# giuliop/AlgoPlonk

Measured on AMD Instinct MI355X. Metric: proofs/sec, higher is better.
Workload: dtype u32x8 (Montgomery Fr/Fp)

## Files before the change

### algoplonk_amd/csrc/apk_api.cpp

```cpp
#include <stdarg.h>
#include <stdio.h>
#include <stdlib.h>
#include <string.h>
#include <atomic>
#include <mutex>
#include <string>
#include <type_traits>

#include <hip/hip_runtime_api.h>

#include "backend.h"
#include "device_sched.h"
#include "ec.h"
#include "kernels_kzg.h"
#include "kernels_kzg_lagrange.h"
#include "plonk_protocol.h"
#include "proof_codec.h"
#include "runtime_env.h"
#include "selftest_ops.h"

namespace apk {

static thread_local std::string g_err;

// ... 490 lines not shown
    if (curve == APK_BLS12_381) return selftest_status(g1_op_t<FrBLS12381, FpBLS12381>(op, p, q, out), "g1", op);
    set_error("unsupported curve: %d", curve);
    return APK_ERR_ARG;
}

int apk_feu_shape(int curve, int field, int* ul, int* ub, uint32_t* headroom) {
    if (!ul || !ub || !headroom) { set_error("null argument"); return APK_ERR_ARG; }
    if (curve == APK_BN254) { field ? feu_shape_t<FpBN254>(ul, ub, headroom) : feu_shape_t<FrBN254>(ul, ub, headroom); return APK_OK; }
    if (curve == APK_BLS12_381) { field ? feu_shape_t<FpBLS12381>(ul, ub, headroom) : feu_shape_t<FrBLS12381>(ul, ub, headroom); return APK_OK; }
    set_error("unsupported curve: %d", curve);
    return APK_ERR_ARG;
}

int apk_host_feu_op(int curve, int field, int op, uint64_t count, const void* in, void* out) {
    if (count && (!in || !out)) { set_error("null argument"); return APK_ERR_ARG; }
    const uint32_t* i = static_cast<const uint32_t*>(in);
    uint32_t* o = static_cast<uint32_t*>(out);
    if (curve == APK_BN254) return field ? host_feu_batch<FpBN254>(op, count, i, o) : host_feu_batch<FrBN254>(op, count, i, o);
    if (curve == APK_BLS12_381) return field ? host_feu_batch<FpBLS12381>(op, count, i, o) : host_feu_batch<FrBLS12381>(op, count, i, o);
    set_error("unsupported curve: %d", curve);
    return APK_ERR_ARG;
}

int apk_device_fe_op(int curve, int field, int op, int device, uint64_t count, const void* a, const void* b, void* out) {
    if (count && (!a || !b || !out)) { set_error("null argument"); return APK_ERR_ARG; }
    if (!seam_args(curve, count, (op >= 0 && op <= 4) || (op >= 10 && op <= 14), op, "field")) return APK_ERR_ARG;
    if (count == 0) return APK_OK;
    runtime_checkpoint();
    return curve == APK_BN254 ? fe_op_device_bn254(device, field, op, count, a, b, out) : fe_op_device_bls12381(device, field, op, count, a, b, out);
}

int apk_device_feu_op(int curve, int field, int op, int device, uint64_t count, const void* in, void* out) {
    if (count && (!in || !out)) { set_error("null argument"); return APK_ERR_ARG; }
    if (!seam_args(curve, count, op >= 0 && op <= 29, op, "unsaturated")) return APK_ERR_ARG;
    if (count == 0) return APK_OK;
    runtime_checkpoint();
    return curve == APK_BN254 ? feu_op_device_bn254(device, field, op, count, in, out) : feu_op_device_bls12381(device, field, op, count, in, out);
}

int apk_device_g1_op(int curve, int op, int device, uint64_t count, const void* p, const void* q, void* out) {
    const bool unary = op == 2 || op == 21;
    if (count && (!p || !out || (!unary && !q))) { set_error("null argument"); return APK_ERR_ARG; }
    if (!seam_args(curve, count, (op >= 0 && op <= 3) || (op >= 10 && op <= 14) || op == 20 || op == 21, op, "g1")) return APK_ERR_ARG;
    if (count == 0) return APK_OK;
    runtime_checkpoint();
    return curve == APK_BN254 ? g1_op_device_bn254(device, op, count, p, q, out) : g1_op_device_bls12381(device, op, count, p, q, out);
}

int apk_g1_sum(int curve, const void* points, uint64_t count, void* out) {
    if (!out || (count && !points)) { set_error("null argument"); return APK_ERR_ARG; }
    if (curve == APK_BN254) return g1_sum_t<FpBN254>(points, count, out);
    if (curve == APK_BLS12_381) return g1_sum_t<FpBLS12381>(points, count, out);
    set_error("unsupported curve: %d", curve);
    return APK_ERR_ARG;
}

int apk_fe_from_be(int curve, int field, const uint8_t* be, void* out) {
    if (!be || !out) { set_error("null argument"); return APK_ERR_ARG; }
    return host_fe_from_be(curve, field, be, out);
}
int apk_fe_to_be(int curve, int field, const void* in, uint8_t* be) {
    if (!be || !in) { set_error("null argument"); return APK_ERR_ARG; }
    return host_fe_to_be(curve, field, in, be);
}

int apk_marshal_proof(const apk_proof* p, uint8_t* out, size_t cap, size_t* len) {
    if (!p || !out || !len) { set_error("null argument"); return APK_ERR_ARG; }
// ... 30 lines not shown
```

### algoplonk_amd/csrc/backend_impl.h

```cpp
#pragma once
#include <hip/hip_runtime.h>
#include <algorithm>
#include <atomic>
#include <chrono>
#include <condition_variable>
#include <memory>
#include <new>
#include <mutex>
#include <string.h>
#include <time.h>
#include <vector>

#include "backend.h"
#include "dev_buf.h"
#include "slot_pinned.h"
#include "msm_run.h"
#include "kzg_run.h"
#include "kernels_ntt.h"
#include "kernels_poly.h"
#include "gang_kernel.h"
#include "kernels_setup.h"
#include "host_msm.h"
#include "slot_gate.h"
#include "gang.h"
// ... 209 lines not shown
        const int log_n = (which ? (int)log_n_ + 2 : (int)log_n_) - sub_log;
        const Fr* tw = which ? (inverse ? ptr<Fr>(twi_4n_) : ptr<Fr>(tw_4n_)) : (inverse ? ptr<Fr>(twi_n_) : ptr<Fr>(twu_n_));
        if (ntt_twu_) tw = which ? (inverse ? ptr<Fr>(twi_4n_x_) : ptr<Fr>(tw_4n_x_)) : (inverse ? ptr<Fr>(twi_n_x_) : ptr<Fr>(twu_n_x_));
        static const int tile_env = env_int("APK_NTT_TILE_LOG", 0, 0, NTT_TILE_LOG);
        static const int stages_env = env_int("APK_NTT_STAGES", 0, 0, NTT_TILE_LOG);
        int tile_log = log_n <= 19 ? 9 : 10;
        int max_s = log_n <= 19 ? 7 : 9;
        if (tile_env) tile_log = tile_env;
        if (stages_env) max_s = stages_env;
        if (tile_log > log_n) tile_log = log_n;
        if (max_s > tile_log) max_s = tile_log;
        const int passes = (log_n + max_s - 1) / max_s;
        bool busy_now = false, busy_foreign = false;
        if (slots_.size() > 2 && log_n >= 17 && log_n <= 19) busy_now = device_load_over(1, &busy_foreign);
        NttBatch nb{};
        for (int i = 0; i < count; i++) { nb.in[i] = ins[i]; nb.out[i] = outs[i]; nb.in_len[i] = in_lens[i]; }
        hipEvent_t e0 = nullptr, e1 = nullptr;
        Slot* owner = nullptr;
        for (Slot* s : slots_) if (s->own_stream == st || (s->side && s->side == st)) owner = s;
        if (passes > 1) {
            if (!owner || log_n > 29) { set_error("ntt: no workspace for this stream"); return APK_ERR_STATE; }
            for (int i = 0; i < count; i++) nb.wide[i] = ptr<FeU<FRP>>(owner->ntt_wide) + ((size_t)i << log_n);
        }
        Slot* timed = stats_on_ ? owner : nullptr;
        if (timed) { e0 = timed->ev2; e1 = timed->ev3; HIPCHK(hipEventRecord(e0, st)); }
        int t0 = 0;
        for (int p = 0; p < passes; p++) {
            int s = (log_n - t0 + (passes - p) - 1) / (passes - p);
            NttPassArgs a;
            a.log_n = log_n; a.tile_log = tile_log; a.t0 = t0; a.t1 = t0 + s;
            a.first = (p == 0); a.last = (p == passes - 1);
            a.out_len = out_len;
            a.tw_shift = sub_log;
            const dim3 grid(1u << (log_n - tile_log), count);
            const size_t lds = ((size_t)1 << tile_log) * sizeof(FeU<FRP>);
            static const int r4_env = env_int("APK_NTT_RADIX4", -1, -1, 1);
            a.radix4 = r4_env >= 0 ? r4_env : (log_n > 19 || (log_n >= 17 && busy_now) ? 1 : 0);
            if (p == 0) { path(P_NTT_SEQ); if (a.radix4) { path(P_NTT_R4); if (r4_env < 0 && log_n <= 19) { path(P_NTT_R4_LOAD); if (busy_foreign) path(P_DEVICE_LOAD); } } }
            static const int thr_env = env_int("APK_NTT_THREADS", 0, 0, NTT_THREADS) & ~63;
            uint32_t threads = NTT_THREADS;
            if (a.radix4) {
                threads = (1u << tile_log) / 4;
                if (threads < 64) threads = 64;
                if (threads > (uint32_t)NTT_THREADS) threads = NTT_THREADS;
            }
            if (thr_env) threads = (uint32_t)thr_env;
            if (ntt_twu_) ntt_pass_kernel<FRP, true><<<grid, threads, lds, st>>>(nb, tw, pre, post, scale, a);
            else ntt_pass_kernel<FRP, false><<<grid, threads, lds, st>>>(nb, tw, pre, post, scale, a);
            KCHK();
            t0 += s;
        }
        if (timed) {
            HIPCHK(hipEventRecord(e1, st));
            HIPCHK(hipEventSynchronize(e1));
            float ms = 0;
            HIPCHK(hipEventElapsedTime(&ms, e0, e1));
            std::lock_guard<std::mutex> g(stats_mu_);
            stats_.ntt_ms += ms;
            stats_.ntt_elements += ((uint64_t)1 << log_n) * count;
        }
        return APK_OK;
    }
    int run_ntt(hipStream_t st, int which, bool inverse, const Fr* in, Fr* out, uint32_t in_len, uint32_t out_len,
                const Fr* pre, const Fr* post, const Fr* scale, int sub_log = 0) {
        return run_ntt_batch(st, which, inverse, 1, &in, &out, &in_len, out_len, pre, post, scale, sub_log);
    }
    int coset_eval(hipStream_t st, int count, const Fr* const* ins, const uint32_t* lens, Fr* const* outs, int cls = 0) {
        if (!sc_.on()) return run_ntt_batch(st, 1, false, count, ins, outs, lens, n4_, ptr<Fr>(coset_pre_), nullptr, nullptr);
        return run_ntt_batch(st, 1, false, count, ins, outs, lens, n4_ >> sc_.glog, ptr<Fr>(sc_.pre[cls]), nullptr, nullptr, sc_.glog);
    }
    int inv_ntt_n(hipStream_t st, const Fr* in, Fr* out) { return run_ntt(st, 0, true, in, out, n_, n_, nullptr, nullptr, ptr<Fr>(scales_)); }
    int coset_ntt_4n(hipStream_t st, const Fr* in, uint32_t len, Fr* out) {
        return run_ntt(st, 1, false, in, out, len, n4_, ptr<Fr>(coset_pre_), nullptr, nullptr);
    }

    int build_lagrange_table(hipStream_t st, const Aff* d_srs, const void* h_lagrange) {
        DevBuf lag;
        CHK(lag.alloc((size_t)(n_ + 3) * sizeof(Aff)));
        if (h_lagrange) HIPCHK(hipMemcpyAsync(lag.p, h_lagrange, (size_t)n_ * sizeof(Aff), hipMemcpyHostToDevice, st));
        else CHK((g1_to_lagrange_dev<FRP, FPP>(d_srs, n_, ptr<Aff>(lag), st)));
        HIPCHK(hipMemcpyAsync(ptr<Aff>(lag) + n_, lag_dk_, sizeof lag_dk_, hipMemcpyHostToDevice, st));
// ... 475 lines not shown
    }
    void drain(Slot* s) {
        if (s->stream) (void)hipStreamSynchronize(s->stream);
        if (s->side_pending && s->side) { (void)hipStreamSynchronize(s->side); s->side_pending = false; }
        (void)hipGetLastError();
    }
    void release(Slot* s, bool ok) {
        if (!ok) drain(s);
        if (s->side_pending) { s->side_pending = false; if (s->own_stream) (void)hipStreamWaitEvent(s->own_stream, s->ev_side, 0); }
        s->own_stream = s->stream = nullptr;
        gate_.release(s->index);
    }
    struct SlotGuard {
        CurveBackend* b; Slot* s; bool ok = false;
        SlotGuard(CurveBackend* b_) : b(b_), s(b_->acquire()) {}
        ~SlotGuard() { b->release(s, ok); }
    };
    struct MaybeGuard {
        CurveBackend* b; Slot* s; bool owned; bool ok = false;
        static Slot* own(CurveBackend* b) { return std::count(b->slots_.begin(), b->slots_.end(), hook_slot()) ? hook_slot() : nullptr; }
        MaybeGuard(CurveBackend* b_) : b(b_), s(own(b_)), owned(s == nullptr) { if (owned) s = b->acquire(); }
        ~MaybeGuard() { if (owned) b->release(s, ok); }
    };
    static bool is_device_ptr(const void* p) {
        hipPointerAttribute_t at{};
        const bool dev = hipPointerGetAttributes(&at, p) == hipSuccess && at.type == hipMemoryTypeDevice;
        if (!dev) (void)hipGetLastError();
        return dev;
    }

    int powers(hipStream_t st, Fr* out, uint32_t count, const Fr& w, const Fr& scale) {
        PowersBatch<FRP> pb{};
        pb.out[0] = out; pb.w[0] = w; pb.scale[0] = scale;
        return klaunch<PowersK<FRP>, 256>(st, dim3(cdiv(cdiv(count, 8), 256), 1), 256, 0, pb, count);
    }
    int powers_batch(hipStream_t st, int k, Fr* const* outs, const Fr* ws, uint32_t count) {
        PowersBatch<FRP> pb{};
        for (int i = 0; i < k; i++) { pb.out[i] = outs[i]; pb.w[i] = ws[i]; pb.scale[i] = Fr::one(); }
        return klaunch<PowersK<FRP>, 256>(st, dim3(cdiv(cdiv(count, 8), 256), k), 256, 0, pb, count);
    }

    int choose_window(int requested, int log_size, int slots = 1) {
        msm_ctx_ = msm_plan_context(FRP::BITS, FPP::N, msm_bases_, log_size, slots, requested, msm_knobs_from_env());
        if (msm_ctx_.rc != APK_OK) { set_error("%s", msm_ctx_.message); return msm_ctx_.rc; }
        return APK_OK;
    }

    int init_msm_only(int device, const void* bases, uint64_t count, int msm_window) override {
        if (!bases || count == 0 || count >= (1ull << 27)) { set_error("msm context: bad base count"); return APK_ERR_ARG; }
        int ndev = 0;
        hipError_t e = hipGetDeviceCount(&ndev);
        if (e != hipSuccess || ndev == 0) { set_error("no HIP device available (%s); libapk has no CPU fallback", e == hipSuccess ? "0 devices" : hipGetErrorString(e)); return APK_ERR_HIP; }
        if (device < 0 || device >= ndev) { set_error("device %d out of range (%d devices)", device, ndev); return APK_ERR_ARG; }
        device_ = device;
        HIPCHK(hipSetDevice(device_));
        { int cus = 0; if (hipDeviceGetAttribute(&cus, hipDeviceAttributeMultiprocessorCount, device_) == hipSuccess && cus > 0) simds_ = 4u * (uint32_t)cus; }
        msm_only_ = true;
        ws_batch_ = 1;
        msm_bases_ = (uint32_t)count;
        n_ = (uint32_t)count;
        int lg = 0;
        while ((1ull << lg) < count) lg++;
        CHK(choose_window(msm_window, lg));
        CHK(set_sort_lds_limits<FRP>(msm_ctx_));
        DevBuf srs;
        CHK(srs.alloc(count * sizeof(Aff)));
        HIPCHK(hipMemcpy(srs.p, bases, count * sizeof(Aff), hipMemcpyHostToDevice));
        CHK((build_tables<FRP, FPP>(nullptr, msm_ctx_, ptr<Aff>(srs), (uint32_t)count, tab_can_)));
        HIPCHK(hipDeviceSynchronize());
        Slot* s = new Slot();
        s->index = slots_.size();
        slots_.push_back(s);
// ... 39 lines not shown
        n_ = (uint32_t)d->n;
        n4_ = 4 * n_;
        log_n_ = 0;
        while ((1u << log_n_) < n_) log_n_++;
        nb_public_ = d->nb_public;
        nb_commit_ = d->nb_commitments;
        for (uint32_t k = 0; k < nb_commit_; k++) {
            cci_[k] = d->commitment_constraint_index[k];
            if ((uint64_t)nb_public_ + cci_[k] >= n_) { set_error("commitment_constraint_index[%u] = %u: row %llu is outside the domain (n = %u)", k, cci_[k], (unsigned long long)nb_public_ + cci_[k], n_); return APK_ERR_ARG; }
        }
        msm_bases_ = n_ + 3;
        CHK(choose_window(d->msm_window, (int)log_n_, d->slots));
        Fr root = root_of_unity();
        const int adicity = FRP::ADICITY;
        omega4_ = root;
        for (int i = 0; i < adicity - (int)log_n_ - 2; i++) omega4_ = Fr::sqr(omega4_);
        omega_ = Fr::sqr(Fr::sqr(omega4_));
        omega_inv_ = Fr::inv(omega_);
        omega4_inv_ = Fr::inv(omega4_);
        shift_ = fr_u64(FRP::COSET_SHIFT);
        shift_inv_ = Fr::inv(shift_);
        n_inv_ = Fr::inv(fr_u64(n_));
        n4_inv_ = Fr::inv(fr_u64(n4_));
        {
            Fr sn = Fr::pow_u64(shift_, n_);
            Fr i4 = Fr::pow_u64(omega4_, n_);
            Fr cur = sn;
            for (int k = 0; k < 4; k++) { zh_inv_[k] = Fr::inv(cur - Fr::one()); cur = cur * i4; }
        }
        hipStream_t st = nullptr;
        const size_t fn = (size_t)n_ * sizeof(Fr), f4 = (size_t)n4_ * sizeof(Fr);
        CHK(tw_n_.alloc(fn / 2)); CHK(twi_n_.alloc(fn / 2)); CHK(tw_4n_.alloc(f4 / 2)); CHK(twi_4n_.alloc(f4 / 2));
        const Fr ru = fr_u64(32);
        HIPCHK(hipFuncSetAttribute(reinterpret_cast<const void*>(&ntt_pass_kernel<FRP, false>), hipFuncAttributeMaxDynamicSharedMemorySize,
                                   (int)(((size_t)1 << NTT_TILE_LOG) * sizeof(FeU<FRP>))));
        HIPCHK(hipFuncSetAttribute(reinterpret_cast<const void*>(&ntt_pass_kernel<FRP, true>), hipFuncAttributeMaxDynamicSharedMemorySize,
                                   (int)(((size_t)1 << NTT_TILE_LOG) * sizeof(FeU<FRP>))));
        CHK(twu_n_.alloc(fn / 2));
        CHK(powers(st, ptr<Fr>(tw_n_), n_ / 2, omega_, Fr::one()));
        CHK(powers(st, ptr<Fr>(twu_n_), n_ / 2, omega_, ru));
        CHK(powers(st, ptr<Fr>(twi_n_), n_ / 2, omega_inv_, ru));
        CHK(powers(st, ptr<Fr>(tw_4n_), n4_ / 2, omega4_, ru));
        CHK(powers(st, ptr<Fr>(twi_4n_), n4_ / 2, omega4_inv_, ru));
        if (env_int("APK_NTT_TWU", 0, 0, 1)) {
            struct { DevBuf* in; DevBuf* out; uint32_t count; } tabs[4] = {{&twu_n_, &twu_n_x_, n_ / 2}, {&twi_n_, &twi_n_x_, n_ / 2},
                                                                            {&tw_4n_, &tw_4n_x_, n4_ / 2}, {&twi_4n_, &twi_4n_x_, n4_ / 2}};
            for (auto& t : tabs) {
                CHK(t.out->alloc((size_t)t.count * sizeof(FeU<FRP>)));
                unpack_table_kernel<FRP><<<cdiv(t.count, 256), 256, 0, st>>>(ptr<Fr>(*t.in), ptr<FeU<FRP>>(*t.out), t.count);
                KCHK();
            }
            ntt_twu_ = true;
        }
        CHK(coset_pre_.alloc((size_t)(n_ + 4) * sizeof(Fr)));
        CHK(powers(st, ptr<Fr>(coset_pre_), n_ + 4, shift_, ru));
        CHK(coset_post_inv_.alloc(f4));
        CHK(powers(st, ptr<Fr>(coset_post_inv_), n4_, shift_inv_, n4_inv_ * ru));
        CHK(scales_.alloc(2 * sizeof(Fr)));
        {
            Fr sc[2] = {n_inv_ * ru, n4_inv_ * ru};
            HIPCHK(hipMemcpy(scales_.p, sc, sizeof sc, hipMemcpyHostToDevice));
        }
        CHK(x4_.alloc(f4));
        CHK(powers(st, ptr<Fr>(x4_), n4_, omega4_, shift_));
        DevBuf srs;
        CHK(srs.alloc((size_t)(n_ + 3) * sizeof(Aff)));
        HIPCHK(hipMemcpy(srs.p, d->srs_g1, (size_t)(n_ + 3) * sizeof(Aff), hipMemcpyHostToDevice));
        CHK((build_tables<FRP, FPP>(st, msm_ctx_, ptr<Aff>(srs), n_ + 3, tab_can_)));
        wires_lag_mode_ = env_int("APK_WIRES_LAGRANGE", -1, -1, 1);
        {
// ... 801 lines not shown
        for (size_t i = 0; i < lin_terms.size(); i++) {
            if (i == LT_QK || (lin_h_done && i >= LT_H1 && i <= LT_H3) || (host_fixed && (i <= LT_QO || i == LT_S3))) continue;
            lp[cnt] = lin_terms[i].com; lk[cnt] = lin_terms[i].coef; cnt++;
        }
        const auto t_lc = std::chrono::steady_clock::now();
        XYZZ<FPP, Fe64<FPP>> sum = host_lincomb_sum<FRP, FPP>(lp, lk, cnt, pool, host_glv);
        if (host_fixed) {
            const Fr fk[5] = {lin_terms[LT_QL].coef, lin_terms[LT_QR].coef, lin_terms[LT_QM].coef, lin_terms[LT_QO].coef, lin_terms[LT_S3].coef};
            vk_fixed_.template accumulate<FRP>(sum, fk);
        }
        if (lin_h_done) sum.add(lin_h);
        {
            using F64 = Fe64<FPP>;
            sum.madd(Affine<FPP, F64>{F64::from(key.qk.x), F64::from(key.qk.y)});
        }
        lin_com = host_xyzz_to_affine<FPP>(sum);
        if (stats_on_) lincomb_ms += std::chrono::duration<double, std::milli>(std::chrono::steady_clock::now() - t_lc).count();
    }
    memcpy(out->zshift_value, &e.zw, sizeof(Fr));
    Fr claimed[6 + APK_MAX_COMMITMENTS] = {lin_sc.lin_z, e.l, e.r, e.o, e.s1, e.s2};
    for (uint32_t k = 0; k < nb_commit_; k++) claimed[6 + k] = e.qcp[k];
    for (uint32_t i = 0; i < 6 + nb_commit_; i++) memcpy(out->claimed_values[i], &claimed[i], sizeof(Fr));
    const Fr gk = Proto::gamma_kzg(zeta, lin_com, lro[0], lro[1], lro[2], key, lin_sc.lin_z, e, gk_raw);
    {
        LinCombArgs<FRP> lc{};
        int c = 0;
        for (const LinTerm& t : lin_terms) { lc.f[c] = t.poly; lc.len[c] = t.len; lc.coef[c] = t.coef; c++; }
        Fr acc = gk;
        auto push = [&](const Fr* f, uint32_t len) { lc.f[c] = f; lc.len[c] = len; lc.coef[c] = acc; c++; acc = acc * gk; };
        push(ptr<Fr>(s.cl), n + 2); push(ptr<Fr>(s.cr), n + 2); push(ptr<Fr>(s.co), n + 2);
        push(ptr<Fr>(s_c_[0]), n); push(ptr<Fr>(s_c_[1]), n);
        for (uint32_t k = 0; k < nb_commit_; k++) push(ptr<Fr>(qcp_c_[k]), n);
        lc.count = c; lc.out_len = n + 3;
        {
            const Fr c32 = fr_u64(32);
            for (int k = 0; k < c; k++) lc.coef[k] = lc.coef[k] * c32;
        }
        CHK((klaunch<LincombK<FRP>, POLY_THREADS>(st, cdiv(n + 3, POLY_THREADS), POLY_THREADS, 0, lc, ptr<Fr>(s.folded))));
        CHK(kzg_quotient(s, ptr<Fr>(s.folded), n + 3, ptr<Fr>(s.pw_z), ptr<Fr>(s.pw_zi), z0, ptr<Fr>(s.q1)));
        MsmBatchArgs a{};
        a.batch = 2;
        a.scalars[0] = s.q1.p; a.len[0] = n + 2; a.offset[0] = 0;
        a.scalars[1] = s.q2.p; a.len[1] = n + 2; a.offset[1] = 0;
        CHK(commit(s, tab_can_, 0, a));
    }
    CHK(sync_results(s));
    store_pt(out->zshift_h, hp[1]);
    store_pt(out->batched_h, hp[0]);
    memcpy(out->gamma, &gamma, sizeof(Fr)); memcpy(out->beta, &beta, sizeof(Fr)); memcpy(out->alpha, &alpha, sizeof(Fr));
    memcpy(out->zeta, &zeta, sizeof(Fr)); memcpy(out->gamma_kzg, &gk, sizeof(Fr));
    mark(3);
    in.ok = true;
    guard.ok = true;
    path(P_PROOFS);
    if (stats_on_) {
        double ms = std::chrono::duration<double, std::milli>(std::chrono::steady_clock::now() - t_start).count();
        std::lock_guard<std::mutex> g(stats_mu_);
        stats_.prove_ms += ms;
        stats_.proofs += 1;
        for (int r = 0; r < 4; r++) stats_.round_ms[r] += phase_ms[r];
        stats_.host_lincomb_ms += lincomb_ms;
    }
    return APK_OK;
}

template <class FRP, class FPP>
// ... 37 lines not shown
    CHK(derr.alloc(4));
    HIPCHK(hipMemcpy(din.p, in, count * nb, hipMemcpyHostToDevice));
    HIPCHK(hipMemset(derr.p, 0, 4));
    g1_decompress_kernel<FRP, FPP, CURVE_ID><<<cdiv(count, 256), 256>>>(ptr<uint8_t>(din), (uint32_t)count, ptr<Aff>(dout), ptr<uint32_t>(derr));
    KCHK();
    uint32_t bad = 0;
    HIPCHK(hipMemcpy(&bad, derr.p, 4, hipMemcpyDeviceToHost));
    if (bad) { set_error("%u compressed point(s) are not valid G1 encodings", bad); return APK_ERR_ARG; }
    HIPCHK(hipMemcpy(out, dout.p, count * sizeof(Aff), hipMemcpyDeviceToHost));
    return APK_OK;
}

template <class FRP, class FPP>
int g1_to_lagrange_dev(const Affine<FPP>* d_in, uint64_t n, Affine<FPP>* d_out, hipStream_t st) {
    using Fr = Fe<FRP>;
    using Aff = Affine<FPP>;
    using Pt = XYZZ<FPP>;
    if (n < 2 || (n & (n - 1)) || n > (1ull << 24)) { set_error("ToLagrangeG1: size must be a power of two in [2, 2^24]"); return APK_ERR_ARG; }
    int log_n = 0;
    while ((1ull << log_n) < n) log_n++;
    Fr root;
    for (int i = 0; i < Fr::N; i++) root.l[i] = FRP::root(i);
    Fr w = Fr::to_mont(root);
    for (int i = 0; i < FRP::ADICITY - log_n; i++) w = Fr::sqr(w);
    Fr winv = Fr::inv(w);
    Fr nn = Fr::zero();
    nn.l[0] = (uint32_t)n;
    Fr ninv = Fr::inv(Fr::to_mont(nn));
    DevBuf work, twi;
    CHK(work.alloc(n * sizeof(Pt)));
    CHK(twi.alloc((n / 2 + 1) * sizeof(Fr)));
    PowersBatch<FRP> pb{};
    pb.out[0] = ptr<Fr>(twi); pb.w[0] = winv; pb.scale[0] = Fr::one();
    powers_kernel<FRP><<<dim3(cdiv(cdiv(n / 2, 8), 256), 1), 256, 0, st>>>(pb, (uint32_t)(n / 2));
    KCHK();
    lagrange_load_kernel<FPP><<<cdiv(n, 256), 256, 0, st>>>(d_in, (uint32_t)n, log_n, ptr<Pt>(work));
    KCHK();
    for (int t = 0; t < log_n; t++) {
        lagrange_stage_kernel<FRP, FPP><<<cdiv(n / 2, 128), 128, 0, st>>>(ptr<Pt>(work), ptr<Fr>(twi), (uint32_t)n, log_n, t);
        KCHK();
    }
    lagrange_finish_kernel<FRP, FPP><<<cdiv(n, 128), 128, 0, st>>>(ptr<Pt>(work), (uint32_t)n, ninv, d_out);
    KCHK();
    HIPCHK(hipStreamSynchronize(st));
    return APK_OK;
}

template <class FRP, class FPP>
int g1_to_lagrange_impl(int device, const void* points, uint64_t n, void* out) {
    using Aff = Affine<FPP>;
    if (n < 2 || (n & (n - 1)) || n > (1ull << 24)) { set_error("ToLagrangeG1: size must be a power of two in [2, 2^24]"); return APK_ERR_ARG; }
    CHK(pick_device(device));
    DevBuf din, dout;
    CHK(din.alloc(n * sizeof(Aff)));
    CHK(dout.alloc(n * sizeof(Aff)));
    HIPCHK(hipMemcpy(din.p, points, n * sizeof(Aff), hipMemcpyHostToDevice));
    CHK((g1_to_lagrange_dev<FRP, FPP>(ptr<Aff>(din), n, ptr<Aff>(dout))));
    HIPCHK(hipMemcpy(out, dout.p, n * sizeof(Aff), hipMemcpyDeviceToHost));
    return APK_OK;
}

template <class P>
__global__ void __launch_bounds__(256) fe_op_kernel(int op, uint32_t count, const Fe<P>* __restrict__ a, const Fe<P>* __restrict__ b,
                                                    Fe<P>* __restrict__ out) {
    const uint32_t i = blockIdx.x * blockDim.x + threadIdx.x;
    if (i < count) (void)fe_op_t<P>(op, a + i, b + i, out + i);
}
// ... 77 lines not shown
```

### algoplonk_amd/csrc/ffu.h

```cpp
#pragma once
#include "ff.h"
#include "ffu_asm.h"

template <class P>
struct FeU {
    static constexpr int L = P::UL;
    static constexpr int B = P::UB;
    static constexpr uint32_t MASK = (1u << B) - 1u;
    static constexpr int N = P::N;
    uint32_t l[L];

    APK_HD static FeU zero() {
        FeU r;
#pragma unroll
        for (int i = 0; i < L; i++) r.l[i] = 0;
        return r;
    }
    APK_HD static FeU one() {
        FeU r;
#pragma unroll
        for (int i = 0; i < L; i++) r.l[i] = P::uone(i);
        return r;
    }
    APK_HD bool is_zero() const {
// ... 231 lines not shown
        }
#pragma unroll
        for (int k = L; k < 2 * L - 1; k++) {
#pragma unroll
            for (int i = k - L + 1; i < L; i++) {
                acc += (uint64_t)a.l[i] * b.l[k - i];
                acc += (uint64_t)c.l[i] * d.l[k - i];
            }
#pragma unroll
            for (int i = k - L + 1; i < L; i++) acc += (uint64_t)m[i] * P::umod(k - i);
            r.l[k - L] = (uint32_t)acc & MASK;
            acc >>= B;
        }
        r.l[L - 1] = (uint32_t)acc;
        return r;
    }

    template <uint32_t K>
    APK_HD static FeU canon(const FeU& a) {
        FeU d;
        uint32_t borrow = 0;
#pragma unroll
        for (int i = 0; i < L; i++) {
            uint32_t t = a.l[i] - kp<K>(i) - borrow;
            borrow = t >> 31;
            d.l[i] = i == L - 1 ? t : (t & MASK);
        }
        FeU r;
#pragma unroll
        for (int i = 0; i < L; i++) r.l[i] = borrow ? a.l[i] : d.l[i];
        if constexpr (K > 1) return canon<K / 2>(r);
        else return r;
    }
    APK_HD bool is_zero_mod_p() const {
        uint32_t z = 0, e = 0;
#pragma unroll
        for (int i = 0; i < L; i++) { z |= l[i]; e |= l[i] ^ P::umod(i); }
        return z == 0 || e == 0;
    }

    APK_HD static FeU unpack(const uint32_t* w) {
        FeU r;
#pragma unroll
        for (int i = 0; i < L; i++) {
            const int bit = i * B, j = bit >> 5, s = bit & 31;
            uint32_t v = j < N ? (w[j] >> s) : 0u;
            if (s + B > 32 && j + 1 < N) v |= w[j + 1] << (32 - s);
            r.l[i] = v & MASK;
        }
        return r;
    }
    APK_HD void pack(uint32_t* w) const {
#pragma unroll
        for (int j = 0; j < N; j++) {
            uint32_t v = 0;
#pragma unroll
            for (int i = 0; i < L; i++) {
                const int lo = i * B - j * 32;
                if (lo > -B && lo < 32) v |= lo >= 0 ? (l[i] << lo) : (l[i] >> (-lo));
            }
            w[j] = v;
        }
    }

    APK_HD static FeU from_fe(const Fe<P>& x) {
        FeU c;
// ... 19 lines not shown
```

### algoplonk_amd/csrc/kernels_ntt.h

```cpp
#pragma once
#include "ff.h"
#include "ffu.h"

namespace apk {

constexpr int NTT_TILE_LOG = 11;
constexpr int NTT_PASS_BITS = 10;
constexpr int NTT_THREADS = 256;

__device__ __forceinline__ uint32_t bitrev32(uint32_t x, int bits) { return __brev(x) >> (32 - bits); }

constexpr int NTT_MAX_BATCH = 4;
constexpr int NTT_ARGS_MAX = 16;
struct NttBatch {
    const void* in[NTT_ARGS_MAX];
    void* out[NTT_ARGS_MAX];
    uint32_t in_len[NTT_ARGS_MAX];
    void* wide[NTT_ARGS_MAX];
};

struct NttPassArgs {
    int log_n;
    int tile_log;
    int t0, t1;
    int first, last;
    uint32_t out_len;
    int radix4;
    int tw_shift;
};

template <class FR, bool TWU = false>
__global__ void __launch_bounds__(NTT_THREADS) ntt_pass_kernel(NttBatch nb, const Fe<FR>* __restrict__ tw,
                                                               const Fe<FR>* __restrict__ pre,
                                                               const Fe<FR>* __restrict__ post,
                                                               const Fe<FR>* __restrict__ scale,
                                                               NttPassArgs a) {
    wave_priority<APK_PRIO_FR>();
    using Fr = Fe<FR>;
    using Fu = FeU<FR>;
    static_assert(Fu::HEADROOM >= 64, "values reach (4 + 2 log2 N) p < 64 p over the stages of a transform (N <= 2^29)");
    extern __shared__ __attribute__((aligned(16))) unsigned char smem_raw[];
    Fu* sm = reinterpret_cast<Fu*>(smem_raw);
    const Fu* __restrict__ twu = reinterpret_cast<const Fu*>(tw);
    auto twiddle = [&](uint32_t idx) -> Fu {
        if constexpr (TWU) return twu[idx];
        else { Fr w = tw[idx]; return Fu::unpack(w.l); }
    };
    Fr* __restrict__ out = reinterpret_cast<Fr*>(nb.out[blockIdx.y]);
    const Fr* __restrict__ in = reinterpret_cast<const Fr*>(nb.in[blockIdx.y]);
    Fu* __restrict__ wide = reinterpret_cast<Fu*>(nb.wide[blockIdx.y]);
    const uint32_t in_len = nb.in_len[blockIdx.y];
    const int s = a.t1 - a.t0;
    const int tile_log = a.tile_log;
    const int clog = tile_log - s;
    const uint32_t C = 1u << clog;
    const uint32_t tile_elems = 1u << tile_log;
    const uint32_t g0 = blockIdx.x << clog;
    const uint32_t lomask = (1u << a.t0) - 1u;

    const uint32_t NT = blockDim.x;
    for (uint32_t e = threadIdx.x; e < tile_elems; e += NT) {
        uint32_t c = e & (C - 1), mid = e >> clog;
        uint32_t g = g0 + c;
        uint32_t idx = ((g >> a.t0) << a.t1) | (mid << a.t0) | (g & lomask);
        Fu v;
        if (a.first) {
            uint32_t src = bitrev32(idx, a.log_n);
            if (src < in_len) {
                Fr raw = in[src];
                v = Fu::unpack(raw.l);
                if (pre) { Fr pw = pre[src]; v = Fu::mul_nr(Fu::unpack(pw.l), v); }
                if (in_len > (1u << a.log_n)) {
                    for (uint32_t s2 = src + (1u << a.log_n); s2 < in_len; s2 += 1u << a.log_n) {
                        Fr raw2 = in[s2];
                        Fu v2 = Fu::unpack(raw2.l);
                        if (pre) { Fr pw = pre[s2]; v2 = Fu::mul_nr(Fu::unpack(pw.l), v2); }
                        v = Fu::add_n(v, v2);
                    }
                    v = Fu::template canon<4>(v);
                }
            } else {
                v = Fu::zero();
            }
        } else {
            v = wide[idx];
        }
        sm[e] = v;
    }
    __syncthreads();
    int q = 0;
    const bool padded = a.first && in_len < (1u << a.log_n);
    const uint32_t nq = tile_elems >> 2;
    for (; a.radix4 && q + 2 <= s; q += 2) {
        const int t = a.t0 + q;
        for (uint32_t u4 = threadIdx.x; u4 < nq; u4 += NT) {
            const uint32_t c = u4 & (C - 1), pr = u4 >> clog;
            const uint32_t low = pr & ((1u << q) - 1u);
            const uint32_t m00 = ((pr >> q) << (q + 2)) | low;
            const uint32_t g = g0 + c;
            const uint32_t imod = (low << a.t0) | (g & lomask);
            const uint32_t e00 = (m00 << clog) | c, st1 = 1u << (q + clog);
            const uint32_t e01 = e00 + st1, e10 = e00 + 2 * st1, e11 = e01 + 2 * st1;
            Fu x0 = sm[e00], x1 = sm[e01], x2 = sm[e10], x3 = sm[e11];
            if (padded && q == 0 && x1.is_zero() && x2.is_zero() && x3.is_zero()) {
                sm[e01] = x0; sm[e10] = x0; sm[e11] = x0;
                continue;
            }
            if (t != 0) {
                const Fu w1 = twiddle((imod << (a.log_n - 1 - t)) << a.tw_shift);
                x1 = Fu::mul_nr(w1, x1);
                x3 = Fu::mul_nr(w1, x3);
            }
            const Fu y0 = Fu::add_n(x0, x1);
            const Fu y1 = Fu::template sub_k<2>(x0, x1);
            Fu y2 = Fu::add_n(x2, x3);
            Fu y3 = Fu::template sub_k<2>(x2, x3);
            const uint32_t k2 = imod << (a.log_n - 2 - t);
            {
                y3 = Fu::mul_nr(twiddle((k2 + (1u << (a.log_n - 2))) << a.tw_shift), y3);
            }
            if (t != 0) {
                y2 = Fu::mul_nr(twiddle(k2 << a.tw_shift), y2);
                sm[e00] = Fu::add_n(y0, y2);
                sm[e10] = Fu::template sub_k<2>(y0, y2);
            } else {
                sm[e00] = Fu::add_n(y0, y2);
                sm[e10] = Fu::template sub_k<4>(y0, y2);
            }
            sm[e01] = Fu::add_n(y1, y3);
            sm[e11] = Fu::template sub_k<2>(y1, y3);
        }
        __syncthreads();
    }
    const uint32_t nbf = tile_elems >> 1;
    for (; q < s; q++) {
        const int t = a.t0 + q;
        for (uint32_t bf = threadIdx.x; bf < nbf; bf += NT) {
            uint32_t c = bf & (C - 1), pr = bf >> clog;
            uint32_t low = pr & ((1u << q) - 1u);
            uint32_t mid0 = ((pr >> q) << (q + 1)) | low;
            uint32_t mid1 = mid0 | (1u << q);
            uint32_t g = g0 + c;
            uint32_t imod = (low << a.t0) | (g & lomask);
            uint32_t tidx = (imod << (a.log_n - 1 - t)) << a.tw_shift;
            uint32_t e0 = (mid0 << clog) | c, e1 = (mid1 << clog) | c;
            Fu u = sm[e0];
            Fu v = sm[e1];
            if (t != 0 && !(padded && v.is_zero())) v = Fu::mul_nr(twiddle(tidx), v);
            sm[e0] = Fu::add_n(u, v);
            sm[e1] = Fu::template sub_k<2>(u, v);
        }
        __syncthreads();
    }
    for (uint32_t e = threadIdx.x; e < tile_elems; e += NT) {
        uint32_t c = e & (C - 1), mid = e >> clog;
        uint32_t g = g0 + c;
        uint32_t idx = ((g >> a.t0) << a.t1) | (mid << a.t0) | (g & lomask);
        Fu v = sm[e];
        if (!a.last) { wide[idx] = v; continue; }
        if (idx >= a.out_len) continue;
        if (post) { Fr pw = post[idx]; v = Fu::mul_nr(Fu::unpack(pw.l), v); }
        if (scale) { Fr sc = scale[0]; v = Fu::mul_nr(Fu::unpack(sc.l), v); }
        v = (post || scale) ? Fu::template canon<1>(v) : Fu::template canon<32>(v);
        Fr o;
        v.pack(o.l);
        out[idx] = o;
    }
}

template <class FR>
__global__ void __launch_bounds__(256) unpack_table_kernel(const Fe<FR>* __restrict__ in, FeU<FR>* __restrict__ out, uint32_t count) {
    const uint32_t i = blockIdx.x * blockDim.x + threadIdx.x;
    if (i >= count) return;
    Fe<FR> v = in[i];
    out[i] = FeU<FR>::unpack(v.l);
}

constexpr int POWERS_MAX_BATCH = 4;
template <class FR>
struct PowersBatch {
    Fe<FR>* out[POWERS_MAX_BATCH];
    Fe<FR> w[POWERS_MAX_BATCH];
    Fe<FR> scale[POWERS_MAX_BATCH];
};
template <class FR>
struct PowersK {
    static __device__ __forceinline__ void run(PowersBatch<FR> pb, uint32_t count) {
        using Fr = Fe<FR>;
        using U = FeU<FR>;
        constexpr uint32_t PER = 8;
        Fr* __restrict__ out = pb.out[blockIdx.y];
        uint32_t t = blockIdx.x * blockDim.x + threadIdx.x;
        uint32_t start = t * PER;
        if (start >= count) return;
        const U wu = U::from_fe(pb.w[blockIdx.y]);
        U r = U::one();
        bool started = false;
        for (int b = 31; b >= 0; b--) {
            if (started) r = U::sqr(r);
            if ((start >> b) & 1u) { r = started ? U::mul(r, wu) : wu; started = true; }
        }
        Fr first = r.to_fe();
        U cur = U::mul(U::unpack(first.l), U::from_fe(pb.scale[blockIdx.y]));
        for (uint32_t k = 0; k < PER && start + k < count; k++) {
            Fr o;
            cur.pack(o.l);
            out[start + k] = o;
            cur = U::mul(wu, cur);
        }
    }
};
template <class FR>
__global__ void __launch_bounds__(256) powers_kernel(PowersBatch<FR> pb, uint32_t count) { PowersK<FR>::run(pb, count); }

}
```

### algoplonk_amd/csrc/kernels_poly.h

```cpp
#pragma once
#include "ff.h"
#include "ffu.h"

namespace apk {

constexpr int POLY_THREADS = 256;
constexpr int SCAN_PER_THREAD = 8;
constexpr int SCAN_BLOCK = POLY_THREADS * SCAN_PER_THREAD;

template <class FR>
struct Fr4 { Fe<FR> v[4]; };

template <class FR>
__global__ void fill_zero_kernel(Fe<FR>* p, uint32_t count) {
    uint32_t i = blockIdx.x * blockDim.x + threadIdx.x;
    if (i < count) p[i] = Fe<FR>::zero();
}

template <class FR>
struct BlindK {
    static __device__ __forceinline__ void run(Fe<FR>* p, uint32_t n, Fr4<FR> b, int d) {
        int i = threadIdx.x;
        if (i < d) {
            p[i] = p[i] - b.v[i];
// ... 403 lines not shown
template <class FR>
struct DerivePowers { const Fe<FR>* in[2]; Fe<FR>* out[2]; int inverse[2]; };
template <class FR>
struct DerivePowersK {
    static __device__ __forceinline__ void run(DerivePowers<FR> a, const Fe<FR>* __restrict__ twu, uint32_t n, uint32_t count) {
        wave_priority<APK_PRIO_FR>();
        using Fr = Fe<FR>;
        using U = FeU<FR>;
        const uint32_t i = blockIdx.x * blockDim.x + threadIdx.x;
        if (i >= count) return;
        const int p = blockIdx.y;
        uint32_t e = i & (n - 1u);
        if (a.inverse[p]) e = (n - e) & (n - 1u);
        const bool neg = e >= n / 2;
        Fr w = twu[e & (n / 2 - 1u)], v = a.in[p][i];
        U r = U::template canon<1>(U::mul_nr(U::unpack(w.l), U::unpack(v.l)));
        Fr o;
        r.pack(o.l);
        if (neg) o = Fr::neg(o);
        a.out[p][i] = o;
    }
};
template <class FR>
__global__ void __launch_bounds__(POLY_THREADS) derive_powers_kernel(DerivePowers<FR> a, const Fe<FR>* __restrict__ twu, uint32_t n, uint32_t count) { DerivePowersK<FR>::run(a, twu, n, count); }

constexpr int LC_MAX = 20;
template <class FR>
struct LinCombArgs {
    const Fe<FR>* f[LC_MAX];
    uint32_t len[LC_MAX];
    Fe<FR> coef[LC_MAX];
    int count;
    uint32_t out_len;
};

template <class FR>
struct LincombK {
    static __device__ __forceinline__ void run(LinCombArgs<FR> a, Fe<FR>* __restrict__ out) {
        wave_priority<APK_PRIO_FR>();
        using Fr = Fe<FR>;
        using U = FeU<FR>;
        static_assert(U::HEADROOM >= 64 && LC_MAX * 2 <= 64, "the sum of LC_MAX products below 2 r each must stay below 64 r");
        uint32_t i = blockIdx.x * blockDim.x + threadIdx.x;
        if (i >= a.out_len) return;
        U acc = U::zero();
        for (int k = 0; k < a.count; k++)
            if (i < a.len[k]) { Fr v = a.f[k][i]; acc = U::add_n(acc, U::mul_nr(U::unpack(a.coef[k].l), U::unpack(v.l))); }
        const U res = U::template canon<32>(acc);
        Fr w;
        res.pack(w.l);
        out[i] = w;
    }
};
template <class FR>
__global__ void __launch_bounds__(POLY_THREADS) lincomb_kernel(LinCombArgs<FR> a, Fe<FR>* __restrict__ out) { LincombK<FR>::run(a, out); }

template <class FR>
struct DivFinishK {
    static __device__ __forceinline__ void run(const Fe<FR>* __restrict__ suffix,
                                                                  const Fe<FR>* __restrict__ zinv_pw, uint32_t len,
                                                                  Fe<FR>* __restrict__ q) {
        wave_priority<APK_PRIO_FR>();
        uint32_t j = blockIdx.x * blockDim.x + threadIdx.x;
        if (j + 1 >= len) return;
        q[j] = suffix[j + 1] * zinv_pw[j + 1];
    }
};
template <class FR>
__global__ void __launch_bounds__(POLY_THREADS) div_finish_kernel(const Fe<FR>* __restrict__ suffix,
                                                                  const Fe<FR>* __restrict__ zinv_pw, uint32_t len,
                                                                  Fe<FR>* __restrict__ q) { DivFinishK<FR>::run(suffix, zinv_pw, len, q); }

template <int DUMMY>
struct TailNonzeroK {
    static __device__ __forceinline__ void run(const uint4* __restrict__ words, uint32_t count4, uint32_t epoch, uint32_t* __restrict__ flag) {
        uint32_t acc = 0;
        for (uint32_t i = blockIdx.x * blockDim.x + threadIdx.x; i < count4; i += gridDim.x * blockDim.x) {
            const uint4 v = words[i];
            acc |= v.x | v.y | v.z | v.w;
        }
        if (__ballot(acc != 0) != 0 && (threadIdx.x & 63) == 0) *reinterpret_cast<volatile uint32_t*>(flag) = epoch;
// ... 17 lines not shown
```

### algoplonk_amd/csrc/selftest_ops.h

```cpp
#pragma once
#include <string.h>
#include <type_traits>

#include "ec.h"

namespace apk {

enum { SELFTEST_OK = 0, SELFTEST_UNKNOWN_OP = 1, SELFTEST_NO_UNSAT = 2 };

template <class P, class = void> struct HasUnsat : std::false_type {};
template <class P> struct HasUnsat<P, std::void_t<decltype(P::UL)>> : std::true_type {};

template <class P>
APK_HD int fe_op_t(int op, const void* a, const void* b, void* out) {
    using F = Fe<P>;
    F x, y, r;
    memcpy(&x, a, sizeof x);
    if (b) memcpy(&y, b, sizeof y); else y = F::zero();
    switch (op) {
        case 0: r = F::add(x, y); break;
        case 1: r = F::sub(x, y); break;
        case 2: r = F::mul(x, y); break;
        case 3: r = F::inv(x); break;
        case 4: r = F::neg(x); break;
// ... 38 lines not shown
        U a, b, c, d, r = U::zero();
        for (int i = 0; i < L; i++) { a.l[i] = in[i]; b.l[i] = in[L + i]; c.l[i] = in[2 * L + i]; d.l[i] = in[3 * L + i]; }
        switch (op) {
            case 0: r = U::reduce_once(a); break;
            case 1: r = U::add(a, b); break;
            case 2: r = U::sub(a, b); break;
            case 3: r = U::neg(a); break;
            case 4: r = U::mul_nr(a, b); break;
            case 5: r = U::mul(a, b); break;
            case 6: r = U::sqr_nr(a); break;
            case 7: r = U::sqr(a); break;
            case 8: r = U::mul2_nr(a, b, c, d); break;
            case 9: r = U::add_n(a, b); break;
            case 10: r = U::triple_n(a); break;
            case 11: r = U::template sub2_k<4>(a, b, c); break;
            case 12: r = U::template sub_k<1>(a, b); break;
            case 13: r = U::template sub_k<2>(a, b); break;
            case 14: r = U::template sub_k<4>(a, b); break;
            case 15: r = U::template sub_k<6>(a, b); break;
            case 16: r = U::template neg_k<1>(a); break;
            case 17: r = U::template neg_k<2>(a); break;
            case 18: r = U::template neg_k<4>(a); break;
            case 19: r = U::template canon<1>(a); break;
            case 20: r = U::template canon<2>(a); break;
            case 21: r = U::template canon<4>(a); break;
            case 22: r = U::template canon<8>(a); break;
            case 23: r = U::template canon<16>(a); break;
            case 24: r = U::template canon<32>(a); break;
            case 25: r.l[0] = a.is_zero_mod_p() ? 1u : 0u; break;
            case 26: r = U::unpack(in); break;
            case 27: a.pack(r.l); break;
            case 28: { Fe<P> x; memcpy(&x, in, sizeof x); r = U::from_fe(x); break; }
            case 29: { const Fe<P> x = a.to_fe(); memcpy(r.l, &x, sizeof x); break; }
            default: return SELFTEST_UNKNOWN_OP;
        }
        for (int i = 0; i < L; i++) out[i] = r.l[i];
        return SELFTEST_OK;
    } else {
        return SELFTEST_NO_UNSAT;
    }
}

template <class FRP, class FPP>
APK_HD int g1_op_t(int op, const void* p, const void* q, void* out) {
    using A = Affine<FPP>;
    using X = XYZZ<FPP>;
    A a, b, r;
    memcpy(&a, p, sizeof a);
    switch (op) {
        case 0: {
            memcpy(&b, q, sizeof b);
            X acc = X::from_affine(a);
            acc.madd(b);
            r = acc.to_affine();
            break;
        }
        case 1: {
            memcpy(&b, q, sizeof b);
            X acc = X::dbl_affine(a);
            acc.madd(a, true);
            X other = X::dbl_affine(b);
            other.madd(b, true);
            acc.add(other);
            r = acc.to_affine();
            break;
        }
// ... 110 lines not shown
```

Measured before the change: 544.6.

## Add quotient-estimate canonicalization, padded-NTT template split, and adaptive powers walk

```diff
diff --git a/algoplonk_amd/csrc/apk_api.cpp b/algoplonk_amd/csrc/apk_api.cpp
--- a/algoplonk_amd/csrc/apk_api.cpp
+++ b/algoplonk_amd/csrc/apk_api.cpp
@@ -546,7 +546,7 @@
 
 int apk_device_feu_op(int curve, int field, int op, int device, uint64_t count, const void* in, void* out) {
     if (count && (!in || !out)) { set_error("null argument"); return APK_ERR_ARG; }
-    if (!seam_args(curve, count, op >= 0 && op <= 29, op, "unsaturated")) return APK_ERR_ARG;
+    if (!seam_args(curve, count, (op >= 0 && op <= 29) || op == 31, op, "unsaturated")) return APK_ERR_ARG;
     if (count == 0) return APK_OK;
     runtime_checkpoint();
     return curve == APK_BN254 ? feu_op_device_bn254(device, field, op, count, in, out) : feu_op_device_bls12381(device, field, op, count, in, out);
diff --git a/algoplonk_amd/csrc/backend_impl.h b/algoplonk_amd/csrc/backend_impl.h
--- a/algoplonk_amd/csrc/backend_impl.h
+++ b/algoplonk_amd/csrc/backend_impl.h
@@ -265,6 +265,8 @@
             a.first = (p == 0); a.last = (p == passes - 1);
             a.out_len = out_len;
             a.tw_shift = sub_log;
+            static const int est_env = env_int("APK_NTT_CANON_EST", 1, 0, 1);
+            a.canon_est = est_env;
             const dim3 grid(1u << (log_n - tile_log), count);
             const size_t lds = ((size_t)1 << tile_log) * sizeof(FeU<FRP>);
             static const int r4_env = env_int("APK_NTT_RADIX4", -1, -1, 1);
@@ -278,8 +280,16 @@
                 if (threads > (uint32_t)NTT_THREADS) threads = NTT_THREADS;
             }
             if (thr_env) threads = (uint32_t)thr_env;
-            if (ntt_twu_) ntt_pass_kernel<FRP, true><<<grid, threads, lds, st>>>(nb, tw, pre, post, scale, a);
-            else ntt_pass_kernel<FRP, false><<<grid, threads, lds, st>>>(nb, tw, pre, post, scale, a);
+            static const int hoist_env = env_int("APK_NTT_PADDED_HOIST", 1, 0, 1);
+            bool padded = !hoist_env;
+            if (p == 0) for (int i = 0; i < count; i++) if (in_lens[i] < (1u << log_n)) padded = true;
+            if (ntt_twu_) {
+                if (padded) ntt_pass_kernel<FRP, true, true><<<grid, threads, lds, st>>>(nb, tw, pre, post, scale, a);
+                else ntt_pass_kernel<FRP, true, false><<<grid, threads, lds, st>>>(nb, tw, pre, post, scale, a);
+            } else {
+                if (padded) ntt_pass_kernel<FRP, false, true><<<grid, threads, lds, st>>>(nb, tw, pre, post, scale, a);
+                else ntt_pass_kernel<FRP, false, false><<<grid, threads, lds, st>>>(nb, tw, pre, post, scale, a);
+            }
             KCHK();
             t0 += s;
         }
@@ -821,12 +831,16 @@
     int powers(hipStream_t st, Fr* out, uint32_t count, const Fr& w, const Fr& scale) {
         PowersBatch<FRP> pb{};
         pb.out[0] = out; pb.w[0] = w; pb.scale[0] = scale;
-        return klaunch<PowersK<FRP>, 256>(st, dim3(cdiv(cdiv(count, 8), 256), 1), 256, 0, pb, count);
+        return klaunch<PowersK<FRP>, 256>(st, dim3(cdiv(cdiv(count, POWERS_WALK), 256), 1), 256, 0, pb, count, POWERS_WALK);
     }
     int powers_batch(hipStream_t st, int k, Fr* const* outs, const Fr* ws, uint32_t count) {
         PowersBatch<FRP> pb{};
         for (int i = 0; i < k; i++) { pb.out[i] = outs[i]; pb.w[i] = ws[i]; pb.scale[i] = Fr::one(); }
-        return klaunch<PowersK<FRP>, 256>(st, dim3(cdiv(cdiv(count, 8), 256), k), 256, 0, pb, count);
+        static const int walk_env = env_int("APK_POWERS_WALK", -1, -1, (int)POWERS_WALK_MAX);
+        uint32_t per = POWERS_WALK;
+        if (walk_env > 0) per = (uint32_t)walk_env;
+        else if (walk_env < 0 && slots_.size() > 2 && device_load_over(1)) per = POWERS_WALK_LOADED;
+        return klaunch<PowersK<FRP>, 256>(st, dim3(cdiv(cdiv(count, per), 256), k), 256, 0, pb, count, per);
     }
 
     int choose_window(int requested, int log_size, int slots = 1) {
@@ -932,10 +946,9 @@
         const size_t fn = (size_t)n_ * sizeof(Fr), f4 = (size_t)n4_ * sizeof(Fr);
         CHK(tw_n_.alloc(fn / 2)); CHK(twi_n_.alloc(fn / 2)); CHK(tw_4n_.alloc(f4 / 2)); CHK(twi_4n_.alloc(f4 / 2));
         const Fr ru = fr_u64(32);
-        HIPCHK(hipFuncSetAttribute(reinterpret_cast<const void*>(&ntt_pass_kernel<FRP, false>), hipFuncAttributeMaxDynamicSharedMemorySize,
-                                   (int)(((size_t)1 << NTT_TILE_LOG) * sizeof(FeU<FRP>))));
-        HIPCHK(hipFuncSetAttribute(reinterpret_cast<const void*>(&ntt_pass_kernel<FRP, true>), hipFuncAttributeMaxDynamicSharedMemorySize,
-                                   (int)(((size_t)1 << NTT_TILE_LOG) * sizeof(FeU<FRP>))));
+        for (const void* fn_ntt : {reinterpret_cast<const void*>(&ntt_pass_kernel<FRP, false, true>), reinterpret_cast<const void*>(&ntt_pass_kernel<FRP, false, false>),
+                                   reinterpret_cast<const void*>(&ntt_pass_kernel<FRP, true, true>), reinterpret_cast<const void*>(&ntt_pass_kernel<FRP, true, false>)})
+            HIPCHK(hipFuncSetAttribute(fn_ntt, hipFuncAttributeMaxDynamicSharedMemorySize, (int)(((size_t)1 << NTT_TILE_LOG) * sizeof(FeU<FRP>))));
         CHK(twu_n_.alloc(fn / 2));
         CHK(powers(st, ptr<Fr>(tw_n_), n_ / 2, omega_, Fr::one()));
         CHK(powers(st, ptr<Fr>(twu_n_), n_ / 2, omega_, ru));
@@ -1803,6 +1816,8 @@
         push(ptr<Fr>(s_c_[0]), n); push(ptr<Fr>(s_c_[1]), n);
         for (uint32_t k = 0; k < nb_commit_; k++) push(ptr<Fr>(qcp_c_[k]), n);
         lc.count = c; lc.out_len = n + 3;
+        static const int lc_est = env_int("APK_LINCOMB_CANON_EST", 1, 0, 1);
+        lc.canon_est = lc_est;
         {
             const Fr c32 = fr_u64(32);
             for (int k = 0; k < c; k++) lc.coef[k] = lc.coef[k] * c32;
@@ -1906,7 +1921,7 @@
     CHK(twi.alloc((n / 2 + 1) * sizeof(Fr)));
     PowersBatch<FRP> pb{};
     pb.out[0] = ptr<Fr>(twi); pb.w[0] = winv; pb.scale[0] = Fr::one();
-    powers_kernel<FRP><<<dim3(cdiv(cdiv(n / 2, 8), 256), 1), 256, 0, st>>>(pb, (uint32_t)(n / 2));
+    powers_kernel<FRP><<<dim3(cdiv(cdiv(n / 2, POWERS_WALK), 256), 1), 256, 0, st>>>(pb, (uint32_t)(n / 2), POWERS_WALK);
     KCHK();
     lagrange_load_kernel<FPP><<<cdiv(n, 256), 256, 0, st>>>(d_in, (uint32_t)n, log_n, ptr<Pt>(work));
     KCHK();
diff --git a/algoplonk_amd/csrc/ffu.h b/algoplonk_amd/csrc/ffu.h
--- a/algoplonk_amd/csrc/ffu.h
+++ b/algoplonk_amd/csrc/ffu.h
@@ -287,6 +287,39 @@
         if constexpr (K > 1) return canon<K / 2>(r);
         else return r;
     }
+    template <uint32_t K2>
+    struct KpTable {
+        uint32_t l[K2][L];
+        constexpr KpTable() : l{} {
+            for (uint32_t j = 0; j < K2; j++) {
+                uint64_t carry = 0;
+                for (int i = 0; i < L; i++) {
+                    const uint64_t t = (uint64_t)j * P::umod(i) + carry;
+                    l[j][i] = i == L - 1 ? (uint32_t)t : (uint32_t)(t & MASK);
+                    carry = t >> B;
+                }
+            }
+        }
+    };
+    template <uint32_t K>
+    APK_HD static FeU canon_est(const FeU& a) {
+        constexpr uint32_t D = P::umod(L - 1) + 1;
+        constexpr uint32_t M = (uint32_t)((1ull << 32) / D);
+        static_assert((uint64_t)2 * K * D <= (1ull << 30), "canon_est: the top limb of a value below 2K*p must stay below 2^30");
+        static_assert((uint64_t)4 * (2 * K + 1) <= D - 1, "canon_est: the estimate must be at most one short");
+        static constexpr KpTable<2 * K> T{};
+        uint32_t q = (uint32_t)(((uint64_t)a.l[L - 1] * M) >> 32);
+        q = q < 2 * K - 1 ? q : 2 * K - 1;
+        FeU d;
+        int32_t carry = 0;
+#pragma unroll
+        for (int i = 0; i < L; i++) {
+            int32_t t = (int32_t)(a.l[i] - T.l[q][i]) + carry;
+            carry = t >> B;
+            d.l[i] = i == L - 1 ? (uint32_t)t : ((uint32_t)t & MASK);
+        }
+        return reduce_once(d);
+    }
     APK_HD bool is_zero_mod_p() const {
         uint32_t z = 0, e = 0;
 #pragma unroll
diff --git a/algoplonk_amd/csrc/kernels_ntt.h b/algoplonk_amd/csrc/kernels_ntt.h
--- a/algoplonk_amd/csrc/kernels_ntt.h
+++ b/algoplonk_amd/csrc/kernels_ntt.h
@@ -27,9 +27,10 @@
     uint32_t out_len;
     int radix4;
     int tw_shift;
-};
-
-template <class FR, bool TWU = false>
+    int canon_est;
+};
+
+template <class FR, bool TWU = false, bool PADDED = true>
 __global__ void __launch_bounds__(NTT_THREADS) ntt_pass_kernel(NttBatch nb, const Fe<FR>* __restrict__ tw,
                                                                const Fe<FR>* __restrict__ pre,
                                                                const Fe<FR>* __restrict__ post,
@@ -89,13 +90,15 @@
     }
     __syncthreads();
     int q = 0;
-    const bool padded = a.first && in_len < (1u << a.log_n);
+    const bool padded = PADDED && a.first && in_len < (1u << a.log_n);
     const uint32_t nq = tile_elems >> 2;
     for (; a.radix4 && q + 2 <= s; q += 2) {
         const int t = a.t0 + q;
+        const int sh1 = a.log_n - 1 - t + a.tw_shift, sh2 = sh1 - 1;
+        const uint32_t quarter = (1u << (a.log_n - 2)) << a.tw_shift, qmask = (1u << q) - 1u;
         for (uint32_t u4 = threadIdx.x; u4 < nq; u4 += NT) {
             const uint32_t c = u4 & (C - 1), pr = u4 >> clog;
-            const uint32_t low = pr & ((1u << q) - 1u);
+            const uint32_t low = pr & qmask;
             const uint32_t m00 = ((pr >> q) << (q + 2)) | low;
             const uint32_t g = g0 + c;
             const uint32_t imod = (low << a.t0) | (g & lomask);
@@ -107,7 +110,7 @@
                 continue;
             }
             if (t != 0) {
-                const Fu w1 = twiddle((imod << (a.log_n - 1 - t)) << a.tw_shift);
+                const Fu w1 = twiddle(imod << sh1);
                 x1 = Fu::mul_nr(w1, x1);
                 x3 = Fu::mul_nr(w1, x3);
             }
@@ -115,12 +118,12 @@
             const Fu y1 = Fu::template sub_k<2>(x0, x1);
             Fu y2 = Fu::add_n(x2, x3);
             Fu y3 = Fu::template sub_k<2>(x2, x3);
-            const uint32_t k2 = imod << (a.log_n - 2 - t);
+            const uint32_t k2 = imod << sh2;
             {
-                y3 = Fu::mul_nr(twiddle((k2 + (1u << (a.log_n - 2))) << a.tw_shift), y3);
+                y3 = Fu::mul_nr(twiddle(k2 + quarter), y3);
             }
             if (t != 0) {
-                y2 = Fu::mul_nr(twiddle(k2 << a.tw_shift), y2);
+                y2 = Fu::mul_nr(twiddle(k2), y2);
                 sm[e00] = Fu::add_n(y0, y2);
                 sm[e10] = Fu::template sub_k<2>(y0, y2);
             } else {
@@ -135,14 +138,16 @@
     const uint32_t nbf = tile_elems >> 1;
     for (; q < s; q++) {
         const int t = a.t0 + q;
+        const int sh = a.log_n - 1 - t + a.tw_shift;
+        const uint32_t qmask = (1u << q) - 1u;
         for (uint32_t bf = threadIdx.x; bf < nbf; bf += NT) {
             uint32_t c = bf & (C - 1), pr = bf >> clog;
-            uint32_t low = pr & ((1u << q) - 1u);
+            uint32_t low = pr & qmask;
             uint32_t mid0 = ((pr >> q) << (q + 1)) | low;
             uint32_t mid1 = mid0 | (1u << q);
             uint32_t g = g0 + c;
             uint32_t imod = (low << a.t0) | (g & lomask);
-            uint32_t tidx = (imod << (a.log_n - 1 - t)) << a.tw_shift;
+            uint32_t tidx = imod << sh;
             uint32_t e0 = (mid0 << clog) | c, e1 = (mid1 << clog) | c;
             Fu u = sm[e0];
             Fu v = sm[e1];
@@ -161,7 +166,7 @@
         if (idx >= a.out_len) continue;
         if (post) { Fr pw = post[idx]; v = Fu::mul_nr(Fu::unpack(pw.l), v); }
         if (scale) { Fr sc = scale[0]; v = Fu::mul_nr(Fu::unpack(sc.l), v); }
-        v = (post || scale) ? Fu::template canon<1>(v) : Fu::template canon<32>(v);
+        v = (post || scale) ? Fu::template canon<1>(v) : a.canon_est ? Fu::template canon_est<32>(v) : Fu::template canon<32>(v);
         Fr o;
         v.pack(o.l);
         out[idx] = o;
@@ -177,6 +182,7 @@
 }
 
 constexpr int POWERS_MAX_BATCH = 4;
+constexpr uint32_t POWERS_WALK = 8, POWERS_WALK_LOADED = 64, POWERS_WALK_MAX = 1024;
 template <class FR>
 struct PowersBatch {
     Fe<FR>* out[POWERS_MAX_BATCH];
@@ -185,14 +191,13 @@
 };
 template <class FR>
 struct PowersK {
-    static __device__ __forceinline__ void run(PowersBatch<FR> pb, uint32_t count) {
+    static __device__ __forceinline__ void run(PowersBatch<FR> pb, uint32_t count, uint32_t per) {
         using Fr = Fe<FR>;
         using U = FeU<FR>;
-        constexpr uint32_t PER = 8;
         Fr* __restrict__ out = pb.out[blockIdx.y];
         uint32_t t = blockIdx.x * blockDim.x + threadIdx.x;
-        uint32_t start = t * PER;
-        if (start >= count) return;
+        if (t >= (count + per - 1) / per) return;
+        uint32_t start = t * per;
         const U wu = U::from_fe(pb.w[blockIdx.y]);
         U r = U::one();
         bool started = false;
@@ -202,7 +207,7 @@
         }
         Fr first = r.to_fe();
         U cur = U::mul(U::unpack(first.l), U::from_fe(pb.scale[blockIdx.y]));
-        for (uint32_t k = 0; k < PER && start + k < count; k++) {
+        for (uint32_t k = 0; k < per && start + k < count; k++) {
             Fr o;
             cur.pack(o.l);
             out[start + k] = o;
@@ -211,6 +216,6 @@
     }
 };
 template <class FR>
-__global__ void __launch_bounds__(256) powers_kernel(PowersBatch<FR> pb, uint32_t count) { PowersK<FR>::run(pb, count); }
+__global__ void __launch_bounds__(256) powers_kernel(PowersBatch<FR> pb, uint32_t count, uint32_t per) { PowersK<FR>::run(pb, count, per); }
 
 }
diff --git a/algoplonk_amd/csrc/kernels_poly.h b/algoplonk_amd/csrc/kernels_poly.h
--- a/algoplonk_amd/csrc/kernels_poly.h
+++ b/algoplonk_amd/csrc/kernels_poly.h
@@ -459,6 +459,7 @@
     Fe<FR> coef[LC_MAX];
     int count;
     uint32_t out_len;
+    int canon_est;
 };
 
 template <class FR>
@@ -473,7 +474,7 @@
         U acc = U::zero();
         for (int k = 0; k < a.count; k++)
             if (i < a.len[k]) { Fr v = a.f[k][i]; acc = U::add_n(acc, U::mul_nr(U::unpack(a.coef[k].l), U::unpack(v.l))); }
-        const U res = U::template canon<32>(acc);
+        const U res = a.canon_est ? U::template canon_est<32>(acc) : U::template canon<32>(acc);
         Fr w;
         res.pack(w.l);
         out[i] = w;
diff --git a/algoplonk_amd/csrc/selftest_ops.h b/algoplonk_amd/csrc/selftest_ops.h
--- a/algoplonk_amd/csrc/selftest_ops.h
+++ b/algoplonk_amd/csrc/selftest_ops.h
@@ -94,6 +94,7 @@
             case 27: a.pack(r.l); break;
             case 28: { Fe<P> x; memcpy(&x, in, sizeof x); r = U::from_fe(x); break; }
             case 29: { const Fe<P> x = a.to_fe(); memcpy(r.l, &x, sizeof x); break; }
+            case 31: r = U::template canon_est<32>(a); break;
             default: return SELFTEST_UNKNOWN_OP;
         }
         for (int i = 0; i < L; i++) out[i] = r.l[i];
```

Result: no change. 546.9 (median of 4 runs) (+0.4%).
